# Keytoyze/Mug-Diffusion

Measured on NVIDIA H100. Metric: denoising-steps/sec, higher is better.
Workload: dtype f32

## Files before the change

### include/mugd.h

```cpp
#ifndef MUGD_H
#define MUGD_H

#include <stdint.h>

#ifdef __cplusplus
extern "C" {
#endif

#define MUGD_ABI_VERSION 13

typedef struct mugd_handle mugd_handle;
typedef struct mugd_plan mugd_plan;

enum mugd_status {
    MUGD_OK = 0,
    MUGD_ERR_INVALID = 1,
    MUGD_ERR_CUDA = 2,
    MUGD_ERR_NO_DEVICE = 3,
    MUGD_ERR_OOM = 4
};

enum mugd_op_kind {
    MUGD_OP_GEMM = 1,
    MUGD_OP_GROUPNORM = 2,
// ... 255 lines not shown
                  void* stream);

int  mugd_grid_scan(mugd_handle* h, const float* times, const int32_t* chart_start, int32_t n_charts,
                    const double* cands, int32_t n_cands,
                    const int32_t* k0, const int32_t* head_len, const double* best_off, const double* best_score,
                    const float* first, const double* head_bpm, const double* head_off,
                    void* workspace, int32_t* out_i, double* out_d, void* stream);

int  mugd_chart_snap(mugd_handle* h, const int32_t* times, const int32_t* chart_start, int32_t n_charts,
                     const double* bpm, const double* offset, const int32_t* offset_is_f32, int64_t* out, void* stream);

int  mugd_remove_mini_jacks(mugd_handle* h, const int32_t* chart_start, int32_t n_charts, double jack_interval,
                            const double* start, const double* end, const uint8_t* is_long, int32_t* x, uint8_t* state,
                            void* workspace, void* stream);

int  mugd_gemm_tc_query(mugd_handle* h, const mugd_gemm* g, int32_t sm_count, int32_t* supported, int32_t* splits,
                        int64_t* workspace_bytes, int32_t* n_tiles);
int  mugd_gemm_tc_variant(const mugd_gemm* g, int32_t sm_count, int32_t* tile_n, int32_t* ctas_per_sm, int32_t* grid_ctas);

int  mugd_set_tc_single_pass_tf32(mugd_handle* h, int enabled);

int  mugd_set_attention_impl(mugd_handle* h, int impl);

int  mugd_debug_set_tc_cost(float kstep128_us, float kstep256_us, float split_us, float two_cta_fixed_us);

int  mugd_debug_set_tc_tile_n(int bn);

int  mugd_debug_set_attention_dump(float* buf);

int  mugd_debug_set_tc_timing(long long* device_buf);

int  mugd_fill_i32(int32_t* dst, int32_t value, void* stream);
int  mugd_abi_sizes(int32_t* out, int32_t n);

#ifdef __cplusplus
}
#endif
#endif
```

### mug_diffusion_b200/csrc/api.cu

```cuda
#include <stdarg.h>
#include <string.h>

#include <vector>

#include "common.cuh"

namespace mugd {

static thread_local char g_err[1024] = "";
bool g_use_pdl = true;

void set_error(const char* fmt, ...) {
    va_list ap;
    va_start(ap, fmt);
    vsnprintf(g_err, sizeof(g_err), fmt, ap);
    va_end(ap);
}

}

struct mugd_handle {
    mugd::DeviceInfo dev;
    int default_gemm_impl = MUGD_GEMM_SIMT;
};
// ... 45 lines not shown
int mugd_create(int device, mugd_handle** out) {
    MUGD_REQUIRE(out, "mugd_create: null out");
    *out = nullptr;
    int n = 0;
    cudaError_t e = cudaGetDeviceCount(&n);
    if (e != cudaSuccess || n <= 0 || device < 0 || device >= n) {
        set_error("mugd_create: no CUDA device %d (count=%d, %s). libmugd has no CPU fallback.", device, n,
                  e == cudaSuccess ? "ok" : cudaGetErrorString(e));
        return MUGD_ERR_NO_DEVICE;
    }
    cudaDeviceProp prop;
    MUGD_CHECK_CUDA(cudaGetDeviceProperties(&prop, device));
    if (prop.major != 9 || prop.minor != 0) {
        set_error("mugd_create: device %d is sm_%d%d; libmugd is built for sm_90a (H100) only", device, prop.major, prop.minor);
        return MUGD_ERR_NO_DEVICE;
    }
    MUGD_CHECK_CUDA(cudaSetDevice(device));
    const int smem_optin = (int)prop.sharedMemPerBlockOptin;
    MUGD_CHECK_CUDA(gemm_tc_allow_smem(smem_optin));
    MUGD_CHECK_CUDA(attention_tc_allow_smem(smem_optin));
    MUGD_CHECK_CUDA(attention_allow_smem(smem_optin));
    MUGD_CHECK_CUDA(s4_allow_smem(smem_optin));
    mugd_handle* h = new mugd_handle();
    h->dev.device = device;
    h->dev.sm_count = prop.multiProcessorCount;
    h->dev.cc_major = prop.major;
    h->dev.cc_minor = prop.minor;
    h->dev.max_smem_optin = smem_optin;
    *out = h;
    return MUGD_OK;
}

void mugd_destroy(mugd_handle* h) { delete h; }

int mugd_device_info(mugd_handle* h, int32_t* sm_count, int32_t* cc_major, int32_t* cc_minor) {
    MUGD_REQUIRE(h, "null handle");
    if (sm_count) *sm_count = h->dev.sm_count;
    if (cc_major) *cc_major = h->dev.cc_major;
    if (cc_minor) *cc_minor = h->dev.cc_minor;
    return MUGD_OK;
}

int mugd_set_gemm_impl(mugd_handle* h, int impl) {
    MUGD_REQUIRE(h, "null handle");
    MUGD_REQUIRE(impl == MUGD_GEMM_SIMT || impl == MUGD_GEMM_TC, "set_gemm_impl: %d", impl);
    h->default_gemm_impl = impl;
    return MUGD_OK;
}

int mugd_set_tc_single_pass_tf32(mugd_handle* h, int enabled) {
    MUGD_REQUIRE(h, "null handle");
    h->dev.tc_single_pass = enabled ? 1 : 0;
    return MUGD_OK;
}

int mugd_set_attention_impl(mugd_handle* h, int impl) {
    MUGD_REQUIRE(h, "null handle");
    h->dev.attention_impl = impl ? 1 : 0;
    return MUGD_OK;
}

int mugd_set_pdl(int enabled) {
    g_use_pdl = enabled != 0;
    return MUGD_OK;
}

int mugd_op_run(mugd_handle* h, const mugd_op* op, void* stream) {
    MUGD_REQUIRE(h && op, "mugd_op_run: null argument");
    return dispatch(h, *op, (cudaStream_t)stream, nullptr);
}

int mugd_plan_create(mugd_handle* h, const mugd_op* ops, int32_t n_ops, mugd_plan** out) {
    MUGD_REQUIRE(h && ops && out && n_ops > 0, "mugd_plan_create: bad arguments");
    mugd_plan* p = new mugd_plan();
    p->h = h;
    p->ops.assign(ops, ops + n_ops);
    *out = p;
    return MUGD_OK;
}

int mugd_plan_run(mugd_plan* p, void* stream) {
// ... 230 lines not shown
```

### mug_diffusion_b200/csrc/common.cuh

```cuda
#pragma once
#include <cuda_runtime.h>
#include <stdint.h>
#include <stdio.h>
#include <string.h>
#include <string>
#include <utility>

#include "../../include/mugd.h"

#if defined(__CUDA_ARCH__) && (__CUDA_ARCH__ != 900)
#error "libmugd is written for sm_90a (H100) only"
#endif

namespace mugd {

void set_error(const char* fmt, ...);

#define MUGD_CHECK_CUDA(expr)                                                             \
    do {                                                                                  \
        cudaError_t _e = (expr);                                                          \
        if (_e != cudaSuccess) {                                                          \
            ::mugd::set_error("%s:%d %s -> %s", __FILE__, __LINE__, #expr,                \
                              cudaGetErrorString(_e));                                    \
            return MUGD_ERR_CUDA;                                                         \
        }                                                                                 \
    } while (0)

#define MUGD_REQUIRE(cond, ...)                                                           \
    do {                                                                                  \
        if (!(cond)) {                                                                    \
            ::mugd::set_error(__VA_ARGS__);                                               \
            return MUGD_ERR_INVALID;                                                      \
        }                                                                                 \
    } while (0)

struct DeviceInfo {
    int device = 0;
    int sm_count = 132;
    int cc_major = 0, cc_minor = 0;
    int max_smem_optin = 0;
    int tc_single_pass = 0;
    int attention_impl = 1;
};

int launch_gemm(const DeviceInfo& dev, const mugd_gemm& g, int default_impl, const mugd_gemm* next, cudaStream_t st, int* launches);
bool gemm_runs_tc(const mugd_gemm& g, int default_impl);
int launch_groupnorm(const DeviceInfo& dev, const mugd_groupnorm& g, cudaStream_t st, int* launches);
int launch_layernorm(const DeviceInfo& dev, const mugd_layernorm& g, cudaStream_t st, int* launches);
int launch_attention(const DeviceInfo& dev, const mugd_attention& a, cudaStream_t st, int* launches);
int launch_s4conv(const DeviceInfo& dev, const mugd_s4conv& s, cudaStream_t st, int* launches);
int launch_ddim_update(const DeviceInfo& dev, const mugd_ddim_update& d, cudaStream_t st, int* launches);
int launch_transpose(const DeviceInfo& dev, const mugd_transpose& t, cudaStream_t st, int* launches);
int launch_copy2d(const DeviceInfo& dev, const mugd_copy2d& c, cudaStream_t st, int* launches);
int launch_step_advance(const DeviceInfo& dev, const mugd_step_advance& a, cudaStream_t st, int* launches);
int launch_notes(const DeviceInfo& dev, const mugd_notes& n, cudaStream_t st, int* launches);
int launch_embed(const DeviceInfo& dev, const mugd_embed& e, cudaStream_t st, int* launches);
int launch_tf32_split(const DeviceInfo& dev, const mugd_tf32_split& s, cudaStream_t st, int* launches);
int launch_posterior(const DeviceInfo& dev, const mugd_posterior& p, cudaStream_t st, int* launches);
int check_stage(const mugd_stage& s, int32_t n_steps);
int launch_stage(const mugd_stage& s, int32_t i, cudaStream_t st);
int check_plms(const mugd_plms& p);
int launch_plms_combine(const mugd_plms& p, int32_t step, int heun, cudaStream_t st);
int check_ddpm(const mugd_ddpm& d);
int launch_ddpm_update(const mugd_ddpm& d, int32_t k, cudaStream_t st);
int check_dpm(const mugd_dpm& d);
int launch_dpm_update(const mugd_dpm& d, cudaStream_t st);
int check_join(const mugd_join& j);
int launch_join(const mugd_join& j, const int32_t* step, cudaStream_t st);
int launch_gemm_tc(const DeviceInfo& dev, const mugd_gemm& g, const mugd_gemm* next, cudaStream_t st, int* launches);
bool gemm_tc_supported(const mugd_gemm& g);

cudaError_t gemm_tc_allow_smem(int bytes);
cudaError_t attention_tc_allow_smem(int bytes);
cudaError_t attention_allow_smem(int bytes);
cudaError_t s4_allow_smem(int bytes);

extern bool g_use_pdl;

#ifdef __CUDACC__
template <typename... KArgs, typename... Args>
inline cudaError_t launch_k(void (*kernel)(KArgs...), dim3 grid, dim3 block, size_t smem, cudaStream_t st, Args&&... args) {
    cudaLaunchConfig_t cfg = {};
    cfg.gridDim = grid;
    cfg.blockDim = block;
    cfg.dynamicSmemBytes = smem;
    cfg.stream = st;
    cudaLaunchAttribute attr[1];
    attr[0].id = cudaLaunchAttributeProgrammaticStreamSerialization;
    attr[0].val.programmaticStreamSerializationAllowed = 1;
    cfg.attrs = attr;
    cfg.numAttrs = g_use_pdl ? 1 : 0;
    return cudaLaunchKernelEx(&cfg, kernel, std::forward<Args>(args)...);
}
template <typename... Kernels>
inline cudaError_t allow_dynamic_smem(int bytes, Kernels... kernels) {
    cudaError_t e = cudaSuccess;
    ((e = (e == cudaSuccess) ? cudaFuncSetAttribute(kernels, cudaFuncAttributeMaxDynamicSharedMemorySize, bytes) : e), ...);
    return e;
}
__device__ __forceinline__ void pdl_wait() { asm volatile("griddepcontrol.wait;" ::: "memory"); }

__device__ __forceinline__ float silu_f(float x) { return x / (1.0f + expf(-x)); }
__device__ __forceinline__ float sigmoid_f(float x) { return 1.0f / (1.0f + expf(-x)); }
__device__ __forceinline__ float gelu_f(float x) { return 0.5f * x * (1.0f + erff(x * 0.70710678118654752440f)); }

__device__ __forceinline__ float4 ld_f4(const float* p) { return *reinterpret_cast<const float4*>(p); }
__device__ __forceinline__ void st_f4(float* p, float4 v) { *reinterpret_cast<float4*>(p) = v; }

template <typename T>
__device__ __forceinline__ T warp_sum(T v) {
#pragma unroll
    for (int o = 16; o > 0; o >>= 1) v += __shfl_xor_sync(0xffffffffu, v, o);
    return v;
}
__device__ __forceinline__ float warp_max(float v) {
// ... 10 lines not shown
```

### mug_diffusion_b200/csrc/gemm_tc.cu

```cuda
#include "gemm_tc.cuh"

namespace mugd {

template <int BN, int EPI>
__global__ void __launch_bounds__(TC_THREADS, 1)
gemm_tc_kernel(const __grid_constant__ CUtensorMap tmA, const __grid_constant__ CUtensorMap tmA1,
               const __grid_constant__ CUtensorMap tmA2, const __grid_constant__ CUtensorMap tmB, const __grid_constant__ CUtensorMap tmWhi,
               const __grid_constant__ CUtensorMap tmWlo, const __grid_constant__ TcParams p) {
    extern __shared__ uint8_t smem_raw[];
    const uint32_t base = (smem_u32(smem_raw) + 1023u) & ~1023u;
    const TcBars<BN> B(base);
    TC_STAMP(p, 0, blockIdx.x == 0 && blockIdx.y == 0 && blockIdx.z == 0);
    if (threadIdx.x < 32) {
        B.init_parallel((int)threadIdx.x);
    } else if (threadIdx.x < 38) {
        const CUtensorMap* m = threadIdx.x == 32 ? &tmA : threadIdx.x == 33 ? &tmA1 : threadIdx.x == 34 ? &tmA2
                             : threadIdx.x == 35 ? &tmB : threadIdx.x == 36 ? &tmWhi : &tmWlo;
        asm volatile("prefetch.tensormap [%0];" ::"l"(reinterpret_cast<uint64_t>(m)) : "memory");
    }
    __syncthreads();
    TC_STAMP(p, 1, blockIdx.x == 0 && blockIdx.y == 0 && blockIdx.z == 0);
    gemm_tc_tile<BN, EPI>(&tmA, &tmA1, &tmA2, &tmB, &tmWhi, &tmWlo, p, blockIdx.x, blockIdx.y, blockIdx.z, base);
}

template <int BN, int EPI>
__global__ void __launch_bounds__(TC_THREADS)
gemm_tc_reduce_kernel(const __grid_constant__ TcParams p) {
    tc_reduce<BN, EPI>(p, blockIdx.x);
}

#ifdef MUGD_TC_TIMELINE
static long long* g_tc_dbg = nullptr;
#endif
static float g_tc_kstep128 = 0.55f;
static float g_tc_split = 3.0f;
static int g_tc_force_bn = 0;

static bool tc_shape_ok(const mugd_gemm& g) {
    if (!(g.conv_mode == MUGD_CONV_NONE || g.conv_mode == MUGD_CONV_SAME || g.conv_mode == MUGD_CONV_DOWN ||
          g.conv_mode == MUGD_CONV_TAPS)) return false;
    if (g.conv_mode == MUGD_CONV_DOWN && g.Lout < 2) return false;
    if (g.K2 % TC_BK != 0 || (g.K2 > 0 && g.conv_mode == MUGD_CONV_DOWN)) return false;
    return g.K % TC_BK == 0 && g.N >= 16 && g.N % 4 == 0;
}

// ... 111 lines not shown
                            "gemm_tc W");
        if (rc != MUGD_OK) return rc;
    }
    TcParams& p = out->p;
    memset(&p, 0, sizeof(p));
    p.hot = h;
    p.hot.single_pass = dev.tc_single_pass ? 1 : 0;
    p.g = g;
    p.ws = (float*)g.workspace;
    p.gy = t.gy;
    p.ln_invK = 1.0 / (double)g.K;
    if (next) {
        p.pf_hi = next->W_hi;
        p.pf_lo = p.hot.single_pass ? nullptr : next->W_lo;
        p.pf_bytes = (int64_t)next->N * ((int64_t)next->taps * next->K + next->K2) * 4;
    }
#ifdef MUGD_TC_TIMELINE
    p.dbg = g_tc_dbg;
#endif
    out->BN = t.BN;
    return MUGD_OK;
}

template <int BN, int EPI>
static int tc_launch(const TcPlanned& pl, cudaStream_t st) {
    const TcParams& p = pl.p;
    const TcParams::Hot& h = p.hot;
    if (h.splits > 1) {
        MUGD_CHECK_CUDA(launch_k(gemm_tc_kernel<BN, TC_E_NONE>, dim3(h.gx, p.gy, h.splits), dim3(TC_THREADS), TcSmem<BN>::TOTAL, st, pl.maps[0],
                                 pl.maps[1], pl.maps[2], pl.maps[3], pl.maps[4], pl.maps[5], p));
        MUGD_CHECK_CUDA(launch_k(gemm_tc_reduce_kernel<BN, EPI>, dim3((unsigned)(h.gx * p.gy * (TC_BM / TC_RED_ROWS<BN>))), dim3(TC_THREADS), 0,
                                 st, p));
        return MUGD_OK;
    }
    MUGD_CHECK_CUDA(launch_k(gemm_tc_kernel<BN, EPI>, dim3(h.gx, p.gy, 1), dim3(TC_THREADS), TcSmem<BN>::TOTAL, st, pl.maps[0], pl.maps[1],
                             pl.maps[2], pl.maps[3], pl.maps[4], pl.maps[5], p));
    return MUGD_OK;
}

template <int BN, int... EPI>
static cudaError_t allow_smem_bn(int bytes, std::integer_sequence<int, EPI...>) {
    return allow_dynamic_smem(bytes, gemm_tc_kernel<BN, EPI>...);
}
cudaError_t gemm_tc_allow_smem(int bytes) {
    const cudaError_t e = allow_smem_bn<64>(bytes, std::make_integer_sequence<int, TC_E_COUNT>{});
    return e != cudaSuccess ? e : allow_smem_bn<128>(bytes, std::make_integer_sequence<int, TC_E_COUNT>{});
}

template <int BN>
static int tc_launch_bn(const TcPlanned& pl, cudaStream_t st) {
    switch (tc_epi_of(pl.p.g)) {
        case TC_E_GEGLU: return tc_launch<BN, TC_E_GEGLU>(pl, st);
        case TC_E_GLU: return tc_launch<BN, TC_E_GLU>(pl, st);
        case TC_E_SILU: return tc_launch<BN, TC_E_SILU>(pl, st);
        case TC_E_GELU: return tc_launch<BN, TC_E_GELU>(pl, st);
        case TC_E_SINK: return tc_launch<BN, TC_E_SINK>(pl, st);
        case TC_E_LN: return tc_launch<BN, TC_E_LN>(pl, st);
        case TC_E_LN_GEGLU: return tc_launch<BN, TC_E_LN_GEGLU>(pl, st);
        default: return tc_launch<BN, TC_E_NONE>(pl, st);
    }
}

int launch_gemm_tc(const DeviceInfo& dev, const mugd_gemm& g, const mugd_gemm* next, cudaStream_t st, int* launches) {
    TcPlanned pl;
    int rc = tc_plan(dev, g, next, &pl);
    if (rc != MUGD_OK) return rc;
    if (pl.BN == 128) rc = tc_launch_bn<128>(pl, st);
    else rc = tc_launch_bn<64>(pl, st);
    if (rc != MUGD_OK) return rc;
    if (launches) *launches += pl.p.hot.splits > 1 ? 2 : 1;
    return MUGD_OK;
}

}

extern "C" int mugd_debug_set_tc_cost(float kstep128_us, float kstep256_us, float split_us, float two_cta_fixed_us) {
    (void)kstep256_us;
    (void)two_cta_fixed_us;
    if (kstep128_us > 0.f) mugd::g_tc_kstep128 = kstep128_us;
    if (split_us > 0.f) mugd::g_tc_split = split_us;
    return MUGD_OK;
}

extern "C" int mugd_debug_set_tc_tile_n(int bn) {
    mugd::g_tc_force_bn = (bn == 64 || bn == 128) ? bn : 0;
    return MUGD_OK;
}

extern "C" int mugd_debug_set_tc_timing(long long* device_buf) {
#ifdef MUGD_TC_TIMELINE
    mugd::g_tc_dbg = device_buf;
    return MUGD_OK;
#else
// ... 42 lines not shown
```

### mug_diffusion_b200/csrc/gemm_tc.cuh

```cuda
#pragma once
#include <cuda.h>
#include <stddef.h>

#include <type_traits>

#include "common.cuh"
#include "wgmma.cuh"

namespace mugd {

constexpr int TC_BM = 128;
constexpr int TC_BK = 32;
constexpr int TC_THREADS = 256;
constexpr uint32_t TC_A_BYTES = TC_BM * TC_BK * 4;

struct TcParams {
    struct Hot {
        int32_t Lrows, Bs;
        int32_t box_l, box_b;
        int32_t tiles_per_sample;
        int32_t it_base, it_rem;
        int32_t it_main;
        int32_t kblocks;
        int32_t total_it;
// ... 136 lines not shown
                        while (m >= smp_end) { ++smp; smp_end += g.Lout; }
                        rvv[u] = ld_f4(rowvec + (int64_t)smp * g.rowvec_b_stride + nn);
                    }
                }
            }
#pragma unroll
            for (int u = 0; u < U; ++u) {
                const int row = row0 + (i0 + u) * RPP;
                const int m = m_base + row;
                const bool ok = FULL || (row < n_rows && col_ok);
                const float4 acc = lds_f4(stage + (uint32_t)(row * SP + c4 * 4) * 4u);
                float2 ln = make_float2(0.f, 1.f);
                if constexpr (MODE == TC_EPI_LN) ln = lds_f2(rowstat + (uint32_t)row * 8u);
                float4 o = make_float4(0.f, 0.f, 0.f, 0.f);
                if (ok) o = tc_finish4<ACT, GATE, MODE == TC_EPI_LN>(g, cp + (int64_t)(i0 + u) * c_step, acc, bia, rvv[u], res[u], cs, ln, m, no);
                if constexpr (MODE == TC_EPI_SINK) tc_row_sink<SEG>(g.row_moments, ok ? m : -1, o);
            }
        }
    };
    if (n_rows >= TC_BM && n0 + BN <= g.N) pass(std::true_type{});
    else pass(std::false_type{});
}

enum TcEpi { TC_E_NONE = 0, TC_E_GEGLU, TC_E_GLU, TC_E_SILU, TC_E_GELU, TC_E_SINK, TC_E_LN, TC_E_LN_GEGLU, TC_E_COUNT };
template <int EPI> struct TcEpiTraits;
template <> struct TcEpiTraits<TC_E_NONE>     { static constexpr int ACT = MUGD_ACT_NONE, GATE = MUGD_GATE_NONE,  MODE = TC_EPI_PLAIN; };
template <> struct TcEpiTraits<TC_E_GEGLU>    { static constexpr int ACT = MUGD_ACT_NONE, GATE = MUGD_GATE_GEGLU, MODE = TC_EPI_PLAIN; };
template <> struct TcEpiTraits<TC_E_GLU>      { static constexpr int ACT = MUGD_ACT_NONE, GATE = MUGD_GATE_GLU,   MODE = TC_EPI_PLAIN; };
template <> struct TcEpiTraits<TC_E_SILU>     { static constexpr int ACT = MUGD_ACT_SILU, GATE = MUGD_GATE_NONE,  MODE = TC_EPI_PLAIN; };
template <> struct TcEpiTraits<TC_E_GELU>     { static constexpr int ACT = MUGD_ACT_GELU, GATE = MUGD_GATE_NONE,  MODE = TC_EPI_PLAIN; };
template <> struct TcEpiTraits<TC_E_SINK>     { static constexpr int ACT = MUGD_ACT_NONE, GATE = MUGD_GATE_NONE,  MODE = TC_EPI_SINK; };
template <> struct TcEpiTraits<TC_E_LN>       { static constexpr int ACT = MUGD_ACT_NONE, GATE = MUGD_GATE_NONE,  MODE = TC_EPI_LN; };
template <> struct TcEpiTraits<TC_E_LN_GEGLU> { static constexpr int ACT = MUGD_ACT_NONE, GATE = MUGD_GATE_GEGLU, MODE = TC_EPI_LN; };

inline int tc_epi_of(const mugd_gemm& g) {
    if (g.ln_stats) return g.gate == MUGD_GATE_GEGLU ? TC_E_LN_GEGLU : TC_E_LN;
    if (g.row_moments) return TC_E_SINK;
    if (g.gate == MUGD_GATE_GEGLU) return TC_E_GEGLU;
    if (g.gate == MUGD_GATE_GLU) return TC_E_GLU;
    if (g.act == MUGD_ACT_SILU) return TC_E_SILU;
    if (g.act == MUGD_ACT_GELU) return TC_E_GELU;
    return TC_E_NONE;
}

__device__ __forceinline__ void tc_tile_rows(const TcParams& p, int by, int& b_base, int& l_base, int& rows_valid) {
    const TcParams::Hot& h = p.hot;
// ... 22 lines not shown
        mbar_init(bars + 8u * t, t < S::STAGES ? 1u : (uint32_t)(TC_THREADS / 32));
        mbar_init_fence();
    }
};

struct TcAFrag {
    uint32_t hi[4][4], lo[4][4];
};
__device__ __forceinline__ void tc_load_split(uint32_t a_tile, int r0, int t, TcAFrag& f) {
#pragma unroll
    for (int kk = 0; kk < 4; ++kk) {
#pragma unroll
        for (int e = 0; e < 4; ++e) {
            const int r = r0 + (e & 1) * 8;
            const int chunk = 2 * kk + (e >> 1);
            const float x = lds_f1(a_tile + (uint32_t)r * 128u + (uint32_t)((chunk ^ (r & 7)) << 4) + (uint32_t)t * 4u);
            const float h = to_tf32(x);
            f.hi[kk][e] = __float_as_uint(h);
            f.lo[kk][e] = __float_as_uint(to_tf32(x - h));
        }
    }
}

template <int BN, int EPI>
__device__ __forceinline__ void gemm_tc_tile(const CUtensorMap* tmA, const CUtensorMap* tmA1, const CUtensorMap* tmA2, const CUtensorMap* tmB,
                                             const CUtensorMap* tmWhi, const CUtensorMap* tmWlo, const TcParams& p, int bx, int by, int bz,
                                             uint32_t base) {
    using S = TcSmem<BN>;
    constexpr int STAGES = S::STAGES;
    constexpr int NACC = BN / 2;
    const TcBars<BN> B(base);
    auto a_raw = [&](int s) { return base + s * S::STAGE_BYTES; };
    auto b_hi = [&](int s) { return base + s * S::STAGE_BYTES + TC_A_BYTES; };
    auto b_lo = [&](int s) { return b_hi(s) + S::B_BYTES; };

    const mugd_gemm& g = p.g;
    const TcParams::Hot& h = p.hot;
    const int warp = threadIdx.x >> 5, lane = threadIdx.x & 31;
    const int n0 = bx * BN;
    int b_base, l_base, rows_valid;
    tc_tile_rows(p, by, b_base, l_base, rows_valid);
    const int m_base = b_base * h.Lrows + l_base;
    const int it_begin = bz * h.it_base + min(bz, h.it_rem);
    const int nit = h.it_base + (bz < h.it_rem ? 1 : 0);
    const uint32_t a_tx = (uint32_t)(h.box_l * h.box_b) * TC_BK * 4;
    const uint32_t w_tx = (h.single_pass ? 1u : 2u) * S::B_BYTES;

// ... 23 lines not shown
            const int pro = nit < STAGES ? nit : STAGES;
            for (int i = 0; i < pro; ++i) issue_w(i);
            pdl_wait();
            for (int i = 0; i < pro; ++i) issue_a(i);
            if (p.pf_bytes > 0) {
                const int64_t ncta = (int64_t)h.gx * p.gy * h.splits;
                const int64_t per = (p.pf_bytes / ncta + 15) & ~(int64_t)15;
                const int64_t off = (((int64_t)bz * p.gy + by) * h.gx + bx) * per;
                const int64_t n = min(per, p.pf_bytes - off);
                if (n > 0) {
                    prefetch_l2(reinterpret_cast<const char*>(p.pf_hi) + off, (uint32_t)n);
                    if (p.pf_lo) prefetch_l2(reinterpret_cast<const char*>(p.pf_lo) + off, (uint32_t)n);
                }
            }
        }
        __syncwarp();
    }

    int epi_step = 0;
    float4 epi_bias = make_float4(0.f, 0.f, 0.f, 0.f), epi_cs = epi_bias;
    double ln_s = 0.0, ln_ss = 0.0;
    {
        pdl_wait();
        if (h.splits == 1) {
            const int nn = n0 + ((int)threadIdx.x % (BN / 4)) * 4;
            if (g.step) epi_step = *g.step;
            if (g.bias && nn < g.N) epi_bias = ld_f4(g.bias + nn);
            if constexpr (TcEpiTraits<EPI>::MODE == TC_EPI_LN) {
                if (nn < g.N) epi_cs = ld_f4(g.ln_colsum + nn);
            }
        }
        if constexpr (TcEpiTraits<EPI>::MODE == TC_EPI_LN) {
            const int rr = (int)threadIdx.x;
            if (rr < TC_BM && rr < rows_valid && m_base + rr < g.M) {
                const double2 mo = *reinterpret_cast<const double2*>(g.ln_stats + (int64_t)m_base * 2 + rr * 2);
                ln_s = mo.x; ln_ss = mo.y;
            }
        }
    }

    const int wg = warp >> 2, g8 = lane >> 2, t4 = lane & 3;
    const int r0 = wg * 64 + (warp & 3) * 16 + g8;
    float acc[NACC];
#pragma unroll
    for (int j = 0; j < NACC; ++j) acc[j] = 0.f;
    TcAFrag f0, f1;
    if (nit > 0) {
// ... 36 lines not shown
        };
        for (int i = 0; i < nit; i += 2) {
            kstep(i, f0, f1);
            if (i + 1 < nit) kstep(i + 1, f1, f0);
        }
    };
    if (h.single_pass) main_loop(std::true_type{});
    else main_loop(std::false_type{});
    wgmma_wait<0>();
    TC_STAMP(p, 2, bx == 0 && by == 0 && bz == 0);
    float2 lnrow = make_float2(0.f, 1.f);
    if constexpr (TcEpiTraits<EPI>::MODE == TC_EPI_LN) lnrow = tc_ln_from_moments(ln_s, ln_ss, p.ln_invK, g.ln_eps);
    __syncthreads();
    constexpr int SP = BN + 4;
#pragma unroll
    for (int j = 0; j < BN / 8; ++j) {
        const int c = j * 8 + 2 * t4;
        sts_f2(base + (uint32_t)(r0 * SP + c) * 4u, acc[4 * j], acc[4 * j + 1]);
        sts_f2(base + (uint32_t)((r0 + 8) * SP + c) * 4u, acc[4 * j + 2], acc[4 * j + 3]);
    }
    if constexpr (TcEpiTraits<EPI>::MODE == TC_EPI_LN) {
        if (threadIdx.x < TC_BM) sts_f2(base + S::TILE_BYTES - 1024u + (uint32_t)threadIdx.x * 8u, lnrow.x, lnrow.y);
    }
    __syncthreads();
    TC_STAMP(p, 3, bx == 0 && by == 0 && bz == 0);
    {
        const float* rowvec = g.rowvec ? g.rowvec + (int64_t)epi_step * g.rowvec_step_stride : nullptr;
        if (h.splits > 1) {
            const int tile_lin = by * h.gx + bx;
            float* wsp = p.ws + ((int64_t)tile_lin * h.splits + bz) * (TC_BM * BN);
            constexpr int C4 = BN / 4;
            constexpr int U = 8;
#pragma unroll 1
            for (int i0 = 0; i0 < TC_BM * C4; i0 += TC_THREADS * U) {
                float4 a4[U];
#pragma unroll
                for (int u = 0; u < U; ++u) {
                    const int idx = i0 + u * TC_THREADS + (int)threadIdx.x;
                    const int row = idx / C4, c4 = idx - row * C4;
                    a4[u] = lds_f4(base + (uint32_t)(row * SP + c4 * 4) * 4u);
                }
#pragma unroll
                for (int u = 0; u < U; ++u) st_f4(wsp + (i0 + u * TC_THREADS + (int)threadIdx.x) * 4, a4[u]);
            }
        } else {
            using E = TcEpiTraits<EPI>;
            tc_store_tile<BN, E::ACT, E::GATE, E::MODE>(g, base, m_base, n0, rows_valid, rowvec, base + S::TILE_BYTES - 1024u, epi_bias, epi_cs);
        }
    }
    TC_STAMP(p, 4, bx == 0 && by == 0 && bz == 0);
}
// ... 76 lines not shown
```

### mug_diffusion_b200/csrc/wgmma.cuh

```cuda
#pragma once
#include <cuda.h>
#include <stdint.h>

#include "common.cuh"

namespace mugd {

#ifdef __CUDACC__
__device__ __forceinline__ uint32_t smem_u32(const void* p) { return (uint32_t)__cvta_generic_to_shared(p); }

__device__ __forceinline__ void mbar_init(uint32_t bar, uint32_t count) {
    asm volatile("mbarrier.init.shared::cta.b64 [%0], %1;" ::"r"(bar), "r"(count) : "memory");
}
__device__ __forceinline__ void mbar_init_fence() { asm volatile("fence.mbarrier_init.release.cluster;" ::: "memory"); }
__device__ __forceinline__ void mbar_expect_tx(uint32_t bar, uint32_t bytes) {
    asm volatile("mbarrier.arrive.expect_tx.shared::cta.b64 _, [%0], %1;" ::"r"(bar), "r"(bytes) : "memory");
}
__device__ __forceinline__ void mbar_arrive(uint32_t bar) {
    asm volatile("mbarrier.arrive.shared::cta.b64 _, [%0];" ::"r"(bar) : "memory");
}
__device__ __forceinline__ void mbar_wait(uint32_t bar, uint32_t parity) {
    uint32_t done = 0;
    long long t0 = 0;
    while (true) {
// ... 5 lines not shown
            : "r"(bar), "r"(parity)
            : "memory");
        if (done) break;
        const long long now = clock64();
        if (t0 == 0) t0 = now;
        else if (now - t0 > 4000000000LL) __trap();
    }
}

__device__ __forceinline__ void tma_load_2d(uint32_t dst, const CUtensorMap* map, uint32_t bar, int c0, int c1) {
    asm volatile(
        "cp.async.bulk.tensor.2d.shared::cluster.global.mbarrier::complete_tx::bytes [%0], [%1, {%3, %4}], [%2];"
        ::"r"(dst), "l"(reinterpret_cast<uint64_t>(map)), "r"(bar), "r"(c0), "r"(c1)
        : "memory");
}
__device__ __forceinline__ void tma_load_3d(uint32_t dst, const CUtensorMap* map, uint32_t bar, int c0, int c1, int c2) {
    asm volatile(
        "cp.async.bulk.tensor.3d.shared::cluster.global.mbarrier::complete_tx::bytes [%0], [%1, {%3, %4, %5}], [%2];"
        ::"r"(dst), "l"(reinterpret_cast<uint64_t>(map)), "r"(bar), "r"(c0), "r"(c1), "r"(c2)
        : "memory");
}
__device__ __forceinline__ void prefetch_l2(const void* p, uint32_t bytes) {
    asm volatile("cp.async.bulk.prefetch.L2.global [%0], %1;" ::"l"(reinterpret_cast<uint64_t>(p)), "r"(bytes) : "memory");
}

__device__ __forceinline__ bool elect_one() {
    uint32_t pred = 0;
    asm volatile(
        "{\n\t.reg .b32 rx;\n\t.reg .pred px;\n\t"
        "elect.sync rx|px, 0xffffffff;\n\t"
        "selp.u32 %0, 1, 0, px;\n\t}"
        : "=r"(pred));
    return pred != 0;
}
__device__ __forceinline__ float to_tf32(float x) {
    uint32_t r;
    asm("cvt.rna.tf32.f32 %0, %1;" : "=r"(r) : "f"(x));
    return __uint_as_float(r);
}

__device__ __forceinline__ float lds_f1(uint32_t addr) {
    float v;
    asm volatile("ld.shared.f32 %0, [%1];" : "=f"(v) : "r"(addr));
    return v;
}
__device__ __forceinline__ float2 lds_f2(uint32_t addr) {
// ... 103 lines not shown
```

### mug_diffusion_b200/lib.py

```python
from __future__ import annotations

import ctypes as C
import os
from typing import Optional

HERE = os.path.dirname(os.path.abspath(__file__))
LIB_PATH = os.environ.get("MUGD_LIB") or os.path.join(HERE, "libmugd.so")

(OP_GEMM, OP_GROUPNORM, OP_LAYERNORM, OP_ATTENTION, OP_S4CONV, OP_DDIM_UPDATE, OP_TRANSPOSE, OP_COPY2D, OP_STEP_ADVANCE, OP_NOTES, OP_EMBED,
 OP_TF32_SPLIT, OP_POSTERIOR) = range(1, 14)
CONV_NONE, CONV_SAME, CONV_DOWN, CONV_UP, CONV_TAPS = range(5)
ACT_NONE, ACT_SILU, ACT_GELU = range(3)
GATE_NONE, GATE_GEGLU, GATE_GLU = range(3)
GEMM_AUTO, GEMM_SIMT, GEMM_TC = range(3)
ABI_VERSION = 13

_f = C.c_void_p


class Gemm(C.Structure):
    _fields_ = [("A", _f), ("lda", C.c_int64), ("W", _f), ("W_hi", _f), ("W_lo", _f), ("bias", _f), ("rowvec", _f),
                ("rowvec_b_stride", C.c_int64), ("rowvec_step_stride", C.c_int64), ("step", _f),
                ("residual", _f), ("ldr", C.c_int64), ("C", _f), ("ldc", C.c_int64),
                ("M", C.c_int32), ("N", C.c_int32), ("K", C.c_int32),
# ... 171 lines not shown
    lib.mugd_abi_sizes.argtypes = [C.POINTER(C.c_int32), C.c_int32]
    if lib.mugd_abi_version() != ABI_VERSION:
        raise MugdError(f"libmugd ABI {lib.mugd_abi_version()} != binding {ABI_VERSION}: rebuild the library")
    sizes = (C.c_int32 * 13)()
    lib.mugd_abi_sizes(sizes, 13)
    mine = [C.sizeof(t) for t in (Op, Gemm, GroupNorm, LayerNorm, Attention, S4Conv, DdimUpdate, Transpose, Copy2D, Notes, Embed, Tf32Split,
                                  Posterior)]
    if list(sizes) != mine:
        raise MugdError(f"struct layout mismatch: C {list(sizes)} vs ctypes {mine}")
    lib.mugd_sample.argtypes = [C.c_void_p, C.POINTER(Op), C.c_int32, C.c_int32, C.c_void_p]
    lib.mugd_sample_staged.argtypes = [C.c_void_p, C.POINTER(Stage), C.POINTER(Op), C.c_int32, C.c_int32, C.c_void_p]
    lib.mugd_sample_plms.argtypes = [C.c_void_p, C.POINTER(Plms), C.c_int32, C.c_int32, C.c_void_p]
    lib.mugd_plms_combine.argtypes = [C.POINTER(Plms), C.c_int32, C.c_int32, C.c_void_p]
    lib.mugd_sample_ddpm.argtypes = [C.c_void_p, C.POINTER(Ddpm), C.c_int32, C.c_int32, C.c_void_p]
    lib.mugd_ddpm_update.argtypes = [C.POINTER(Ddpm), C.c_void_p]
    lib.mugd_sample_dpm.argtypes = [C.c_void_p, C.POINTER(Dpm), C.c_int32, C.c_int32, C.c_void_p]
    lib.mugd_dpm_update.argtypes = [C.POINTER(Dpm), C.c_void_p]
    lib.mugd_stochastic_encode.argtypes = [C.POINTER(QEncode), C.c_void_p]
    lib.mugd_sample_join.argtypes = [C.c_void_p, C.POINTER(Join), C.POINTER(Op), C.c_int32, C.c_int32, C.c_int32, C.c_void_p]
    lib.mugd_plan_save.argtypes = [C.c_void_p, C.POINTER(Region), C.c_int32, C.c_char_p]
    lib.mugd_plan_load.argtypes = [C.c_void_p, C.c_char_p, C.POINTER(Region), C.c_int32, C.POINTER(C.c_void_p)]
    lib.mugd_set_tc_single_pass_tf32.argtypes = [C.c_void_p, C.c_int]
    lib.mugd_set_attention_impl.argtypes = [C.c_void_p, C.c_int]
    lib.mugd_debug_set_tc_tile_n.argtypes = [C.c_int]
    lib.mugd_debug_set_tc_cost.argtypes = [C.c_float, C.c_float, C.c_float, C.c_float]
    if os.environ.get("MUGD_TC_COST"):
        lib.mugd_debug_set_tc_cost(*([float(v) for v in os.environ["MUGD_TC_COST"].split(",")] + [0.0] * 4)[:4])
    if os.environ.get("MUGD_TC_TILE"):
        lib.mugd_debug_set_tc_tile_n(int(os.environ["MUGD_TC_TILE"]))
    if os.environ.get("MUGD_TC_BN"):
        lib.mugd_debug_set_tc_tile_n(int(os.environ["MUGD_TC_BN"]))
    if os.environ.get("MUGD_PDL") in ("0", "1"):
        lib.mugd_set_pdl(int(os.environ["MUGD_PDL"]))
    _lib = lib
    return lib


def check(rc: int, what: str = ""):
    if rc != 0:
        msg = load().mugd_last_error().decode(errors="replace")
        if rc == 4:
            import torch
            raise torch.cuda.OutOfMemoryError(f"{what}: {msg}")
        raise MugdError(f"{what} failed (status {rc}): {msg}")


EXPORTED_SYMBOLS = [
    "mugd_abi_version", "mugd_last_error", "mugd_create", "mugd_destroy", "mugd_device_info", "mugd_set_gemm_impl",
    "mugd_op_run", "mugd_plan_create", "mugd_plan_run", "mugd_plan_capture", "mugd_plan_replay",
    "mugd_plan_launch_count", "mugd_plan_destroy", "mugd_s4_kernel_gen", "mugd_fill_i32", "mugd_abi_sizes", "mugd_gemm_tc_query",
    "mugd_set_pdl", "mugd_set_tc_single_pass_tf32", "mugd_set_attention_impl", "mugd_debug_set_tc_tile_n", "mugd_debug_set_tc_cost", "mugd_gemm_tc_variant",
    "mugd_debug_set_attention_dump", "mugd_debug_set_tc_timing", "mugd_sample", "mugd_plan_save", "mugd_plan_load", "mugd_plan_regions", "mugd_plan_ops",
    "mugd_melspec", "mugd_grid_scan", "mugd_chart_snap", "mugd_remove_mini_jacks",
    "mugd_sample_staged", "mugd_sample_plms", "mugd_plms_combine",
    "mugd_sample_ddpm", "mugd_ddpm_update", "mugd_stochastic_encode", "mugd_sample_join",
    "mugd_sample_dpm", "mugd_dpm_update",
]
```

Before: 243.0.

## Reduce split-K GEMM partials through distributed shared memory in a CTA cluster

For tensor-core GEMMs with two K-splits, the two split CTAs are launched as a cluster along z. Each CTA reads its peer's accumulator tile through distributed shared memory and applies the fused epilogue to its own half of the rows. This replaces the global workspace write plus the separate reduce kernel launch. The cost is cluster scheduling constraints, which are checked against an occupancy query run at handle creation, and two extra cluster barriers.

```diff
diff --git a/include/mugd.h b/include/mugd.h
--- a/include/mugd.h
+++ b/include/mugd.h
@@ -301,6 +301,8 @@
 
 int  mugd_set_attention_impl(mugd_handle* h, int impl);
 
+int  mugd_set_tc_cluster_reduce(mugd_handle* h, int enabled);
+
 int  mugd_debug_set_tc_cost(float kstep128_us, float kstep256_us, float split_us, float two_cta_fixed_us);
 
 int  mugd_debug_set_tc_tile_n(int bn);
diff --git a/mug_diffusion_b200/csrc/api.cu b/mug_diffusion_b200/csrc/api.cu
--- a/mug_diffusion_b200/csrc/api.cu
+++ b/mug_diffusion_b200/csrc/api.cu
@@ -91,6 +91,7 @@
     MUGD_CHECK_CUDA(attention_allow_smem(smem_optin));
     MUGD_CHECK_CUDA(s4_allow_smem(smem_optin));
     mugd_handle* h = new mugd_handle();
+    gemm_tc_cluster_caps(h->dev);
     h->dev.device = device;
     h->dev.sm_count = prop.multiProcessorCount;
     h->dev.cc_major = prop.major;
@@ -126,6 +127,12 @@
 int mugd_set_attention_impl(mugd_handle* h, int impl) {
     MUGD_REQUIRE(h, "null handle");
     h->dev.attention_impl = impl ? 1 : 0;
+    return MUGD_OK;
+}
+
+int mugd_set_tc_cluster_reduce(mugd_handle* h, int enabled) {
+    MUGD_REQUIRE(h, "null handle");
+    h->dev.tc_cluster_reduce = enabled ? 1 : 0;
     return MUGD_OK;
 }
 
diff --git a/mug_diffusion_b200/csrc/common.cuh b/mug_diffusion_b200/csrc/common.cuh
--- a/mug_diffusion_b200/csrc/common.cuh
+++ b/mug_diffusion_b200/csrc/common.cuh
@@ -41,6 +41,8 @@
     int max_smem_optin = 0;
     int tc_single_pass = 0;
     int attention_impl = 1;
+    int tc_cluster_reduce = 1;
+    int16_t tc_pair_cap[2][8] = {};
 };
 
 int launch_gemm(const DeviceInfo& dev, const mugd_gemm& g, int default_impl, const mugd_gemm* next, cudaStream_t st, int* launches);
@@ -71,6 +73,7 @@
 bool gemm_tc_supported(const mugd_gemm& g);
 
 cudaError_t gemm_tc_allow_smem(int bytes);
+void gemm_tc_cluster_caps(DeviceInfo& dev);
 cudaError_t attention_tc_allow_smem(int bytes);
 cudaError_t attention_allow_smem(int bytes);
 cudaError_t s4_allow_smem(int bytes);
@@ -79,18 +82,34 @@
 
 #ifdef __CUDACC__
 template <typename... KArgs, typename... Args>
-inline cudaError_t launch_k(void (*kernel)(KArgs...), dim3 grid, dim3 block, size_t smem, cudaStream_t st, Args&&... args) {
+inline cudaError_t launch_k_cluster(void (*kernel)(KArgs...), dim3 grid, dim3 block, size_t smem, cudaStream_t st, unsigned cluster_z,
+                                    Args&&... args) {
     cudaLaunchConfig_t cfg = {};
     cfg.gridDim = grid;
     cfg.blockDim = block;
     cfg.dynamicSmemBytes = smem;
     cfg.stream = st;
-    cudaLaunchAttribute attr[1];
-    attr[0].id = cudaLaunchAttributeProgrammaticStreamSerialization;
-    attr[0].val.programmaticStreamSerializationAllowed = 1;
+    cudaLaunchAttribute attr[2];
+    int n = 0;
+    if (g_use_pdl) {
+        attr[n].id = cudaLaunchAttributeProgrammaticStreamSerialization;
+        attr[n].val.programmaticStreamSerializationAllowed = 1;
+        ++n;
+    }
+    if (cluster_z > 1) {
+        attr[n].id = cudaLaunchAttributeClusterDimension;
+        attr[n].val.clusterDim.x = 1;
+        attr[n].val.clusterDim.y = 1;
+        attr[n].val.clusterDim.z = cluster_z;
+        ++n;
+    }
     cfg.attrs = attr;
-    cfg.numAttrs = g_use_pdl ? 1 : 0;
+    cfg.numAttrs = n;
     return cudaLaunchKernelEx(&cfg, kernel, std::forward<Args>(args)...);
+}
+template <typename... KArgs, typename... Args>
+inline cudaError_t launch_k(void (*kernel)(KArgs...), dim3 grid, dim3 block, size_t smem, cudaStream_t st, Args&&... args) {
+    return launch_k_cluster(kernel, grid, block, smem, st, 1u, std::forward<Args>(args)...);
 }
 template <typename... Kernels>
 inline cudaError_t allow_dynamic_smem(int bytes, Kernels... kernels) {
diff --git a/mug_diffusion_b200/csrc/gemm_tc.cu b/mug_diffusion_b200/csrc/gemm_tc.cu
--- a/mug_diffusion_b200/csrc/gemm_tc.cu
+++ b/mug_diffusion_b200/csrc/gemm_tc.cu
@@ -2,7 +2,7 @@
 
 namespace mugd {
 
-template <int BN, int EPI>
+template <int BN, int EPI, bool CLUSTER>
 __global__ void __launch_bounds__(TC_THREADS, 1)
 gemm_tc_kernel(const __grid_constant__ CUtensorMap tmA, const __grid_constant__ CUtensorMap tmA1,
                const __grid_constant__ CUtensorMap tmA2, const __grid_constant__ CUtensorMap tmB, const __grid_constant__ CUtensorMap tmWhi,
@@ -20,7 +20,7 @@
     }
     __syncthreads();
     TC_STAMP(p, 1, blockIdx.x == 0 && blockIdx.y == 0 && blockIdx.z == 0);
-    gemm_tc_tile<BN, EPI>(&tmA, &tmA1, &tmA2, &tmB, &tmWhi, &tmWlo, p, blockIdx.x, blockIdx.y, blockIdx.z, base);
+    gemm_tc_tile<BN, EPI, CLUSTER>(&tmA, &tmA1, &tmA2, &tmB, &tmWhi, &tmWlo, p, blockIdx.x, blockIdx.y, blockIdx.z, base);
 }
 
 template <int BN, int EPI>
@@ -178,42 +178,86 @@
     return MUGD_OK;
 }
 
+static_assert(TC_E_COUNT == 8, "DeviceInfo::tc_pair_cap is [2][TC_E_COUNT]");
+
+static bool tc_use_cluster(const DeviceInfo& dev, const TcPlanned& pl) {
+    const TcParams::Hot& h = pl.p.hot;
+    if (!dev.tc_cluster_reduce || h.splits != 2) return false;
+    const int cap = dev.tc_pair_cap[pl.BN == 128 ? 1 : 0][tc_epi_of(pl.p.g)];
+    const int pairs = h.gx * pl.p.gy;
+    return cap > 0 && (pairs + cap - 1) / cap <= (2 * pairs + dev.sm_count - 1) / dev.sm_count;
+}
+
 template <int BN, int EPI>
-static int tc_launch(const TcPlanned& pl, cudaStream_t st) {
+static int tc_launch(const TcPlanned& pl, bool cluster, cudaStream_t st) {
     const TcParams& p = pl.p;
     const TcParams::Hot& h = p.hot;
+    if (cluster) {
+        MUGD_CHECK_CUDA(launch_k_cluster(gemm_tc_kernel<BN, EPI, true>, dim3(h.gx, p.gy, h.splits), dim3(TC_THREADS), TcSmem<BN>::TOTAL, st,
+                                         (unsigned)h.splits, pl.maps[0], pl.maps[1], pl.maps[2], pl.maps[3], pl.maps[4], pl.maps[5], p));
+        return MUGD_OK;
+    }
     if (h.splits > 1) {
-        MUGD_CHECK_CUDA(launch_k(gemm_tc_kernel<BN, TC_E_NONE>, dim3(h.gx, p.gy, h.splits), dim3(TC_THREADS), TcSmem<BN>::TOTAL, st, pl.maps[0],
-                                 pl.maps[1], pl.maps[2], pl.maps[3], pl.maps[4], pl.maps[5], p));
+        MUGD_CHECK_CUDA(launch_k(gemm_tc_kernel<BN, TC_E_NONE, false>, dim3(h.gx, p.gy, h.splits), dim3(TC_THREADS), TcSmem<BN>::TOTAL, st,
+                                 pl.maps[0], pl.maps[1], pl.maps[2], pl.maps[3], pl.maps[4], pl.maps[5], p));
         MUGD_CHECK_CUDA(launch_k(gemm_tc_reduce_kernel<BN, EPI>, dim3((unsigned)(h.gx * p.gy * (TC_BM / TC_RED_ROWS<BN>))), dim3(TC_THREADS), 0,
                                  st, p));
         return MUGD_OK;
     }
-    MUGD_CHECK_CUDA(launch_k(gemm_tc_kernel<BN, EPI>, dim3(h.gx, p.gy, 1), dim3(TC_THREADS), TcSmem<BN>::TOTAL, st, pl.maps[0], pl.maps[1],
+    MUGD_CHECK_CUDA(launch_k(gemm_tc_kernel<BN, EPI, false>, dim3(h.gx, p.gy, 1), dim3(TC_THREADS), TcSmem<BN>::TOTAL, st, pl.maps[0], pl.maps[1],
                              pl.maps[2], pl.maps[3], pl.maps[4], pl.maps[5], p));
     return MUGD_OK;
 }
 
 template <int BN, int... EPI>
 static cudaError_t allow_smem_bn(int bytes, std::integer_sequence<int, EPI...>) {
-    return allow_dynamic_smem(bytes, gemm_tc_kernel<BN, EPI>...);
+    const cudaError_t e = allow_dynamic_smem(bytes, gemm_tc_kernel<BN, EPI, false>...);
+    return e != cudaSuccess ? e : allow_dynamic_smem(bytes, gemm_tc_kernel<BN, EPI, true>...);
 }
 cudaError_t gemm_tc_allow_smem(int bytes) {
     const cudaError_t e = allow_smem_bn<64>(bytes, std::make_integer_sequence<int, TC_E_COUNT>{});
     return e != cudaSuccess ? e : allow_smem_bn<128>(bytes, std::make_integer_sequence<int, TC_E_COUNT>{});
 }
 
+template <int BN, int... EPI>
+static void cluster_caps_bn(DeviceInfo& dev, std::integer_sequence<int, EPI...>) {
+    void (*kernels[])(CUtensorMap, CUtensorMap, CUtensorMap, CUtensorMap, CUtensorMap, CUtensorMap, TcParams) = {gemm_tc_kernel<BN, EPI, true>...};
+    for (int e = 0; e < (int)sizeof...(EPI); ++e) {
+        cudaLaunchConfig_t cfg = {};
+        cfg.gridDim = dim3(1, 1, 2);
+        cfg.blockDim = dim3(TC_THREADS);
+        cfg.dynamicSmemBytes = TcSmem<BN>::TOTAL;
+        cudaLaunchAttribute attr[1];
+        attr[0].id = cudaLaunchAttributeClusterDimension;
+        attr[0].val.clusterDim.x = 1;
+        attr[0].val.clusterDim.y = 1;
+        attr[0].val.clusterDim.z = 2;
+        cfg.attrs = attr;
+        cfg.numAttrs = 1;
+        int n = 0;
+        if (cudaOccupancyMaxActiveClusters(&n, kernels[e], &cfg) != cudaSuccess) {
+            n = 0;
+            (void)cudaGetLastError();
+        }
+        dev.tc_pair_cap[BN == 128 ? 1 : 0][e] = (int16_t)(n < 0 ? 0 : n > 32767 ? 32767 : n);
+    }
+}
+void gemm_tc_cluster_caps(DeviceInfo& dev) {
+    cluster_caps_bn<64>(dev, std::make_integer_sequence<int, TC_E_COUNT>{});
+    cluster_caps_bn<128>(dev, std::make_integer_sequence<int, TC_E_COUNT>{});
+}
+
 template <int BN>
-static int tc_launch_bn(const TcPlanned& pl, cudaStream_t st) {
+static int tc_launch_bn(const TcPlanned& pl, bool cluster, cudaStream_t st) {
     switch (tc_epi_of(pl.p.g)) {
-        case TC_E_GEGLU: return tc_launch<BN, TC_E_GEGLU>(pl, st);
-        case TC_E_GLU: return tc_launch<BN, TC_E_GLU>(pl, st);
-        case TC_E_SILU: return tc_launch<BN, TC_E_SILU>(pl, st);
-        case TC_E_GELU: return tc_launch<BN, TC_E_GELU>(pl, st);
-        case TC_E_SINK: return tc_launch<BN, TC_E_SINK>(pl, st);
-        case TC_E_LN: return tc_launch<BN, TC_E_LN>(pl, st);
-        case TC_E_LN_GEGLU: return tc_launch<BN, TC_E_LN_GEGLU>(pl, st);
-        default: return tc_launch<BN, TC_E_NONE>(pl, st);
+        case TC_E_GEGLU: return tc_launch<BN, TC_E_GEGLU>(pl, cluster, st);
+        case TC_E_GLU: return tc_launch<BN, TC_E_GLU>(pl, cluster, st);
+        case TC_E_SILU: return tc_launch<BN, TC_E_SILU>(pl, cluster, st);
+        case TC_E_GELU: return tc_launch<BN, TC_E_GELU>(pl, cluster, st);
+        case TC_E_SINK: return tc_launch<BN, TC_E_SINK>(pl, cluster, st);
+        case TC_E_LN: return tc_launch<BN, TC_E_LN>(pl, cluster, st);
+        case TC_E_LN_GEGLU: return tc_launch<BN, TC_E_LN_GEGLU>(pl, cluster, st);
+        default: return tc_launch<BN, TC_E_NONE>(pl, cluster, st);
     }
 }
 
@@ -221,10 +265,11 @@
     TcPlanned pl;
     int rc = tc_plan(dev, g, next, &pl);
     if (rc != MUGD_OK) return rc;
-    if (pl.BN == 128) rc = tc_launch_bn<128>(pl, st);
-    else rc = tc_launch_bn<64>(pl, st);
+    const bool cluster = tc_use_cluster(dev, pl);
+    if (pl.BN == 128) rc = tc_launch_bn<128>(pl, cluster, st);
+    else rc = tc_launch_bn<64>(pl, cluster, st);
     if (rc != MUGD_OK) return rc;
-    if (launches) *launches += pl.p.hot.splits > 1 ? 2 : 1;
+    if (launches) *launches += (pl.p.hot.splits > 1 && !cluster) ? 2 : 1;
     return MUGD_OK;
 }
 
diff --git a/mug_diffusion_b200/csrc/gemm_tc.cuh b/mug_diffusion_b200/csrc/gemm_tc.cuh
--- a/mug_diffusion_b200/csrc/gemm_tc.cuh
+++ b/mug_diffusion_b200/csrc/gemm_tc.cuh
@@ -182,6 +182,62 @@
     else pass(std::false_type{});
 }
 
+template <int BN, int ACT, int GATE, int MODE>
+__device__ __forceinline__ void tc_cluster_store(const mugd_gemm& g, uint32_t stage, int splits, int rank, int m_base, int n0, int rows_valid,
+                                                 const float* rowvec, uint32_t rowstat, float4 bia, float4 cs) {
+    constexpr int SP = BN + 4;
+    constexpr int C4 = BN / 4;
+    constexpr int RPP = TC_THREADS / C4;
+    constexpr int SEG = C4 < 32 ? C4 : 32;
+    const int c4 = (int)threadIdx.x % C4;
+    const int nn = n0 + c4 * 4;
+    const bool col_ok = nn < g.N;
+    const int no = (GATE == MUGD_GATE_NONE) ? nn : (nn >> 1);
+    const int r_lo = rank * TC_BM / splits, r_hi = (rank + 1) * TC_BM / splits;
+    const int r_end = min(r_hi, min(rows_valid, g.M - m_base));
+    const uint32_t col_off = (uint32_t)(c4 * 4) * 4u;
+    {
+        constexpr int UR = 8, ZU = 2;
+        uint32_t peer[ZU];
+#pragma unroll
+        for (int z = 0; z < ZU; ++z) peer[z] = z < splits ? cluster_map(stage, (uint32_t)z) : 0u;
+#pragma unroll 1
+        for (int rb = r_lo; rb < r_hi; rb += RPP * UR) {
+            float4 res[UR], rvv[UR], t[UR][ZU];
+#pragma unroll
+            for (int u = 0; u < UR; ++u) {
+                const int row = rb + u * RPP + (int)threadIdx.x / C4;
+                const int m = m_base + row;
+                const bool ok = row < r_end && col_ok;
+                res[u] = rvv[u] = make_float4(0.f, 0.f, 0.f, 0.f);
+                if (ok && GATE == MUGD_GATE_NONE && g.residual) res[u] = ld_f4(g.residual + (int64_t)m * g.ldr + nn);
+                if (ok && rowvec) rvv[u] = ld_f4(rowvec + (int64_t)(m / g.Lout) * g.rowvec_b_stride + nn);
+#pragma unroll
+                for (int z = 0; z < ZU; ++z) {
+                    t[u][z] = make_float4(0.f, 0.f, 0.f, 0.f);
+                    if (ok && z < splits) t[u][z] = ld_cluster_f4(peer[z] + (uint32_t)(row * SP) * 4u + col_off);
+                }
+            }
+#pragma unroll
+            for (int u = 0; u < UR; ++u) {
+                const int row = rb + u * RPP + (int)threadIdx.x / C4;
+                const int m = m_base + row;
+                const bool ok = row < r_end && col_ok;
+                float4 acc = make_float4(0.f, 0.f, 0.f, 0.f);
+#pragma unroll
+                for (int z = 0; z < ZU; ++z) { acc.x += t[u][z].x; acc.y += t[u][z].y; acc.z += t[u][z].z; acc.w += t[u][z].w; }
+                float2 ln = make_float2(0.f, 1.f);
+                if constexpr (MODE == TC_EPI_LN) {
+                    if (ok) ln = lds_f2(rowstat + (uint32_t)row * 8u);
+                }
+                float4 o = make_float4(0.f, 0.f, 0.f, 0.f);
+                if (ok) o = tc_finish4<ACT, GATE, MODE == TC_EPI_LN>(g, g.C + (int64_t)m * g.ldc + no, acc, bia, rvv[u], res[u], cs, ln, m, no);
+                if constexpr (MODE == TC_EPI_SINK) tc_row_sink<SEG>(g.row_moments, ok ? m : -1, o);
+            }
+        }
+    }
+}
+
 enum TcEpi { TC_E_NONE = 0, TC_E_GEGLU, TC_E_GLU, TC_E_SILU, TC_E_GELU, TC_E_SINK, TC_E_LN, TC_E_LN_GEGLU, TC_E_COUNT };
 template <int EPI> struct TcEpiTraits;
 template <> struct TcEpiTraits<TC_E_NONE>     { static constexpr int ACT = MUGD_ACT_NONE, GATE = MUGD_GATE_NONE,  MODE = TC_EPI_PLAIN; };
@@ -250,7 +306,7 @@
     }
 }
 
-template <int BN, int EPI>
+template <int BN, int EPI, bool CLUSTER>
 __device__ __forceinline__ void gemm_tc_tile(const CUtensorMap* tmA, const CUtensorMap* tmA1, const CUtensorMap* tmA2, const CUtensorMap* tmB,
                                              const CUtensorMap* tmWhi, const CUtensorMap* tmWlo, const TcParams& p, int bx, int by, int bz,
                                              uint32_t base) {
@@ -320,7 +376,7 @@
     double ln_s = 0.0, ln_ss = 0.0;
     {
         pdl_wait();
-        if (h.splits == 1) {
+        if (CLUSTER || h.splits == 1) {
             const int nn = n0 + ((int)threadIdx.x % (BN / 4)) * 4;
             if (g.step) epi_step = *g.step;
             if (g.bias && nn < g.N) epi_bias = ld_f4(g.bias + nn);
@@ -403,11 +459,17 @@
     if constexpr (TcEpiTraits<EPI>::MODE == TC_EPI_LN) {
         if (threadIdx.x < TC_BM) sts_f2(base + S::TILE_BYTES - 1024u + (uint32_t)threadIdx.x * 8u, lnrow.x, lnrow.y);
     }
-    __syncthreads();
+    if constexpr (CLUSTER) cluster_sync();
+    else __syncthreads();
     TC_STAMP(p, 3, bx == 0 && by == 0 && bz == 0);
     {
         const float* rowvec = g.rowvec ? g.rowvec + (int64_t)epi_step * g.rowvec_step_stride : nullptr;
-        if (h.splits > 1) {
+        if constexpr (CLUSTER) {
+            using E = TcEpiTraits<EPI>;
+            tc_cluster_store<BN, E::ACT, E::GATE, E::MODE>(g, base, h.splits, bz, m_base, n0, rows_valid, rowvec, base + S::TILE_BYTES - 1024u,
+                                                           epi_bias, epi_cs);
+            cluster_sync();
+        } else if (h.splits > 1) {
             const int tile_lin = by * h.gx + bx;
             float* wsp = p.ws + ((int64_t)tile_lin * h.splits + bz) * (TC_BM * BN);
             constexpr int C4 = BN / 4;
diff --git a/mug_diffusion_b200/csrc/wgmma.cuh b/mug_diffusion_b200/csrc/wgmma.cuh
--- a/mug_diffusion_b200/csrc/wgmma.cuh
+++ b/mug_diffusion_b200/csrc/wgmma.cuh
@@ -51,6 +51,20 @@
 }
 __device__ __forceinline__ void prefetch_l2(const void* p, uint32_t bytes) {
     asm volatile("cp.async.bulk.prefetch.L2.global [%0], %1;" ::"l"(reinterpret_cast<uint64_t>(p)), "r"(bytes) : "memory");
+}
+
+__device__ __forceinline__ void cluster_sync() {
+    asm volatile("barrier.cluster.arrive.release;\n\tbarrier.cluster.wait.acquire;" ::: "memory");
+}
+__device__ __forceinline__ uint32_t cluster_map(uint32_t saddr, uint32_t rank) {
+    uint32_t r;
+    asm volatile("mapa.shared::cluster.u32 %0, %1, %2;" : "=r"(r) : "r"(saddr), "r"(rank));
+    return r;
+}
+__device__ __forceinline__ float4 ld_cluster_f4(uint32_t caddr) {
+    float4 v;
+    asm volatile("ld.shared::cluster.v4.f32 {%0, %1, %2, %3}, [%4];" : "=f"(v.x), "=f"(v.y), "=f"(v.z), "=f"(v.w) : "r"(caddr) : "memory");
+    return v;
 }
 
 __device__ __forceinline__ bool elect_one() {
diff --git a/mug_diffusion_b200/lib.py b/mug_diffusion_b200/lib.py
--- a/mug_diffusion_b200/lib.py
+++ b/mug_diffusion_b200/lib.py
@@ -217,6 +217,7 @@
     lib.mugd_plan_load.argtypes = [C.c_void_p, C.c_char_p, C.POINTER(Region), C.c_int32, C.POINTER(C.c_void_p)]
     lib.mugd_set_tc_single_pass_tf32.argtypes = [C.c_void_p, C.c_int]
     lib.mugd_set_attention_impl.argtypes = [C.c_void_p, C.c_int]
+    lib.mugd_set_tc_cluster_reduce.argtypes = [C.c_void_p, C.c_int]
     lib.mugd_debug_set_tc_tile_n.argtypes = [C.c_int]
     lib.mugd_debug_set_tc_cost.argtypes = [C.c_float, C.c_float, C.c_float, C.c_float]
     if os.environ.get("MUGD_TC_COST"):
@@ -244,7 +245,7 @@
     "mugd_abi_version", "mugd_last_error", "mugd_create", "mugd_destroy", "mugd_device_info", "mugd_set_gemm_impl",
     "mugd_op_run", "mugd_plan_create", "mugd_plan_run", "mugd_plan_capture", "mugd_plan_replay",
     "mugd_plan_launch_count", "mugd_plan_destroy", "mugd_s4_kernel_gen", "mugd_fill_i32", "mugd_abi_sizes", "mugd_gemm_tc_query",
-    "mugd_set_pdl", "mugd_set_tc_single_pass_tf32", "mugd_set_attention_impl", "mugd_debug_set_tc_tile_n", "mugd_debug_set_tc_cost", "mugd_gemm_tc_variant",
+    "mugd_set_pdl", "mugd_set_tc_single_pass_tf32", "mugd_set_attention_impl", "mugd_set_tc_cluster_reduce", "mugd_debug_set_tc_tile_n", "mugd_debug_set_tc_cost", "mugd_gemm_tc_variant",
     "mugd_debug_set_attention_dump", "mugd_debug_set_tc_timing", "mugd_sample", "mugd_plan_save", "mugd_plan_load", "mugd_plan_regions", "mugd_plan_ops",
     "mugd_melspec", "mugd_grid_scan", "mugd_chart_snap", "mugd_remove_mini_jacks",
     "mugd_sample_staged", "mugd_sample_plms", "mugd_plms_combine",
```

Result: no change. 244.3, median of 6 (+0.5%).
